# FelipeMartins96/rsoccer-isaac-cleanrl

Measured on NVIDIA B200. Metric: vss_env_steps_per_s, higher is better.
Workload: dtype f32

## Files before the change

### rsoccer_isaac_cleanrl_b200/csrc/vss_lane.cuh

```cuda
#pragma once
#include <stdint.h>
#include <math.h>
#include <string.h>
#if defined(__CUDACC__)
#include <cuda_bf16.h>
#endif

#include "../../include/vss_b200.h"

#if defined(__CUDACC__)
#define VSS_HD __host__ __device__ __forceinline__
#define VSS_HD_COLD inline __host__ __device__ __noinline__
#else
#define VSS_HD inline
#define VSS_HD_COLD inline
#endif

#ifndef VSS_INTEG_UNROLL
#define VSS_INTEG_UNROLL 1
#endif

namespace vss {

constexpr int INTEG_UNROLL = VSS_INTEG_UNROLL;
// ... 590 lines not shown
      const float p_dist = S[(W_PREV + 1 + r) * LDS];
      const float dist = norm2(fsub(x, bx), fsub(y, by));
      rew[4 * r + 2] = fmul(fsub(p_dist, dist), P.w_move);
    }
  }
  if (P.w_energy > 0.0f) {
#pragma unroll
    for (int r = 0; r < 6; ++r) {
      const float al = S[(11 + 9 * r) * LDS], ar = S[(12 + 9 * r) * LDS];
      rew[4 * r + 3] = fmul(-fmul(fadd(fabsf(al), fabsf(ar)), 0.5f), P.w_energy);
    }
  }
}

VSS_HD_COLD void reset_lane(float* S, const DevParams& P, const RngKey& key) {
  const uint32_t ep = fbits(S[VSS_W_EPISODE * LDS]);
  float px[7], py[7];
#pragma unroll 1
  for (uint32_t attempt = 0; attempt < (uint32_t)RESET_MAX_ATTEMPTS; ++attempt) {
    uint32_t u[16];
#pragma unroll
    for (uint32_t b = 0; b < 4; ++b) {
      const U4 g = rng_block(key, ep, STREAM_RESET_POS, (attempt << 2) | b);
      u[4 * b] = g.x; u[4 * b + 1] = g.y; u[4 * b + 2] = g.z; u[4 * b + 3] = g.w;
    }
#pragma unroll
    for (int e = 0; e < 7; ++e) {
      px[e] = fmul(fsub(u01(u[2 * e]), 0.5f), P.reset_sx);
      py[e] = fmul(fsub(u01(u[2 * e + 1]), 0.5f), P.reset_sy);
    }
    bool too_close = false;
#pragma unroll
    for (int a = 0; a < 7; ++a)
#pragma unroll
      for (int b = a + 1; b < 7; ++b) {
        const float dx = fsub(px[a], px[b]), dy = fsub(py[a], py[b]);
        too_close |= ffma(dy, dy, fmul(dx, dx)) < P.min_d2;
      }
    if (!too_close) break;
  }
  const U4 m0 = rng_block(key, ep, STREAM_RESET_MISC, 0), m1 = rng_block(key, ep, STREAM_RESET_MISC, 1);
  const uint32_t m[8] = {m0.x, m0.y, m0.z, m0.w, m1.x, m1.y, m1.z, m1.w};
  S[0] = px[0]; S[LDS] = py[0];
  S[2 * LDS] = fmul(fsub(u01(m[6]), 0.5f), P.ball_speed);
  S[3 * LDS] = fmul(fsub(u01(m[7]), 0.5f), P.ball_speed);
#pragma unroll
  for (int r = 0; r < 6; ++r) {
    float* b = S + (4 + 9 * r) * LDS;
    const float yaw = fsub(fmul(u01(m[r]), 6.283185307179586f), 3.141592653589793f);
    b[0] = px[1 + r]; b[LDS] = py[1 + r];
    b[2 * LDS] = 0.0f; b[3 * LDS] = 0.0f;
    b[4 * LDS] = cosf(yaw); b[5 * LDS] = sinf(yaw);
    b[6 * LDS] = 0.0f; b[7 * LDS] = 0.0f; b[8 * LDS] = 0.0f;
  }
  S[VSS_W_EPISODE * LDS] = bitsf(ep + 1u);
}

VSS_HD void ou_block(float a4[4], const DevParams& P, const RngKey& key, uint32_t step, uint32_t b) {
  const U4 g = rng_block(key, step, STREAM_OU, b);
  const uint32_t u[4] = {g.x, g.y, g.z, g.w};
#pragma unroll
  for (int h = 0; h < 2; ++h) {
    const float rad = fsqrt(fmul(-2.0f, logf(u01_open(u[2 * h]))));
    const float ang = fmul(6.283185307179586f, u01(u[2 * h + 1]));
    const float z[2] = {fmul(rad, cosf(ang)), fmul(rad, sinf(ang))};
#pragma unroll
    for (int c = 0; c < 2; ++c) {
      float& v = a4[2 * h + c];
      v = clampf(fadd(fsub(v, fmul(P.ou_theta, v)), fmul(P.ou_sigma, z[c])), -1.0f, 1.0f);
    }
  }
}
VSS_HD void ou_lane(float a[VSS_ACT_PER_FIELD], const DevParams& P, const RngKey& key, uint32_t step) {
#pragma unroll
  for (uint32_t b = 0; b < 3; ++b) ou_block(a + 4 * b, P, key, step, b);
}


#if defined(__CUDA_ARCH__)
VSS_HD F4 ld4(const float* p) { const float4 v = *reinterpret_cast<const float4*>(p); return F4{v.x, v.y, v.z, v.w}; }
VSS_HD void st4(float* p, const F4& v) { *reinterpret_cast<float4*>(p) = make_float4(v.x, v.y, v.z, v.w); }
VSS_HD void st4_stream(float* p, const F4& v) { __stcs(reinterpret_cast<float4*>(p), make_float4(v.x, v.y, v.z, v.w)); }
VSS_HD float ldg(const float* p) { return __ldg(p); }
VSS_HD void st_bf16x4(void* base, long long off, const F4& v) {
  const uint32_t lo = (uint32_t)__bfloat16_as_ushort(__float2bfloat16_rn(v.x)) |
                      ((uint32_t)__bfloat16_as_ushort(__float2bfloat16_rn(v.y)) << 16);
  const uint32_t hi = (uint32_t)__bfloat16_as_ushort(__float2bfloat16_rn(v.z)) |
                      ((uint32_t)__bfloat16_as_ushort(__float2bfloat16_rn(v.w)) << 16);
  *reinterpret_cast<uint2*>(reinterpret_cast<unsigned short*>(base) + off) = make_uint2(lo, hi);
}
#else
VSS_HD F4 ld4(const float* p) { return F4{p[0], p[1], p[2], p[3]}; }
VSS_HD void st4(float* p, const F4& v) { p[0] = v.x; p[1] = v.y; p[2] = v.z; p[3] = v.w; }
VSS_HD void st4_stream(float* p, const F4& v) { st4(p, v); }
VSS_HD float ldg(const float* p) { return *p; }
VSS_HD uint32_t bf16_rne(float f) {
  const uint32_t u = fbits(f);
  if ((u & 0x7FFFFFFFu) > 0x7F800000u) return 0x7FFFu;
  return (u + 0x7FFFu + ((u >> 16) & 1u)) >> 16;
}
VSS_HD void st_bf16x4(void* base, long long off, const F4& v) {
  unsigned short* p = reinterpret_cast<unsigned short*>(base) + off;
  p[0] = (unsigned short)bf16_rne(v.x); p[1] = (unsigned short)bf16_rne(v.y);
  p[2] = (unsigned short)bf16_rne(v.z); p[3] = (unsigned short)bf16_rne(v.w);
}
#endif

constexpr int VIEW_FULL = -1;
constexpr int VIEW_MATCH = 3;

struct StepArgs {
  float* state; long long n, ld; unsigned long long goff;
  long long env_begin;
  uint32_t seed_lo, seed_hi;
  unsigned long long* step_ctr;
  uint32_t grid;
  const float* actions;
  const float* inject;
  long long* reset_buf;
  float* obs;
  float* term_obs;
  float* rew;
  uint8_t* timeout;
  float* progress_f;
  const float* policy_action; float* action_buf; float* reward_v; long long* done_v;
  float* ep_ret; int* ep_len; float* ret_ret; int* ret_len;
  void* obs_bf16; float* done_f; float* timeout_f;
  void* packed;
  int fpw;
  int stagger_ns;
  int team_mode[2];
  const float* team_action[2];
  void* team_rows[2];
  long long count_envs, n_matches;
  vss_match_board* board;
};

template <int VIEW>
struct ViewShape {
  static constexpr int F4_PER = (VIEW == VIEW_FULL || VIEW == VIEW_MATCH) ? F4_PER_FIELD
                                                                          : (VIEW == VSS_VIEW_DMA ? 3 * F4_PER_ROW : F4_PER_ROW);
  static constexpr int AGENTS = VIEW == VSS_VIEW_DMA ? 3 : 1;
};

VSS_HD uint32_t step_index(const StepArgs& a) {
#if defined(__CUDA_ARCH__)
  return (uint32_t)__ldcg(a.step_ctr);
#else
  return (uint32_t)*a.step_ctr;
#endif
}

VSS_HD RngKey make_key(const StepArgs& a, long long env) {
  const unsigned long long gid = a.goff + (unsigned long long)env;
  return RngKey{a.seed_lo, a.seed_hi, (uint32_t)gid, (uint32_t)(gid >> 32)};
}

VSS_HD void load_state(float* S, const float* state, long long ld, long long env) {
  const float* src = state + env;
#pragma unroll
  for (int w = 0; w < VSS_STATE_WORDS; ++w) S[w * LDS] = ldg(src + (long long)w * ld);
}
VSS_HD void store_state(const float* S, float* state, long long ld, long long env) {
  float* dst = state + env;
#pragma unroll
  for (int w = 0; w < VSS_STATE_WORDS; ++w) dst[(long long)w * ld] = S[w * LDS];
}

VSS_HD bool match_needs_ou(const StepArgs& a) {
  return a.team_mode[0] == VSS_TEAM_OU || a.team_mode[0] == VSS_TEAM_SA || a.team_mode[1] == VSS_TEAM_OU ||
         a.team_mode[1] == VSS_TEAM_SA;
}
VSS_HD float match_slot(const StepArgs& a, long long env, int s, float prev, float ou) {
  const int t = s >= 6 ? 1 : 0, k = s - 6 * t;
  switch (a.team_mode[t]) {
    case VSS_TEAM_ZERO: return fmul(prev, 0.0f);
    case VSS_TEAM_OU: return ou;
    case VSS_TEAM_SA: return k < 2 ? a.team_action[t][2 * env + k] : ou;
    case VSS_TEAM_CMA:
    case VSS_TEAM_DMA: return a.team_action[t][6 * env + k];
    default: return prev;
  }
}

template <int VIEW>
VSS_HD void lane_phase1a(float* S, long long env, const StepArgs& a, const DevParams& P, const RngKey& key) {
  load_state(S, a.state, a.ld, env);
  float act[VSS_ACT_PER_FIELD];
  {
    const float* ap = (VIEW == VIEW_FULL ? a.actions : a.action_buf) + env * VSS_ACT_PER_FIELD;
#pragma unroll
    for (int q = 0; q < 3; ++q) {
      const F4 v = ld4(ap + 4 * q);
      act[4 * q] = v.x; act[4 * q + 1] = v.y; act[4 * q + 2] = v.z; act[4 * q + 3] = v.w;
    }
  }
  if (VIEW == VIEW_MATCH) {
    float ou[VSS_ACT_PER_FIELD];
#pragma unroll
    for (int q = 0; q < VSS_ACT_PER_FIELD; ++q) ou[q] = act[q];
    if (match_needs_ou(a)) ou_lane(ou, P, key, step_index(a));
#pragma unroll
    for (int q = 0; q < VSS_ACT_PER_FIELD; ++q) act[q] = match_slot(a, env, q, act[q], ou[q]);
    float* ap = a.action_buf + env * VSS_ACT_PER_FIELD;
#pragma unroll
    for (int q = 0; q < 3; ++q) st4(ap + 4 * q, F4{act[4 * q], act[4 * q + 1], act[4 * q + 2], act[4 * q + 3]});
  } else if (VIEW != VIEW_FULL) {
    ou_lane(act, P, key, step_index(a));
    if (VIEW == VSS_VIEW_SA) {
      act[0] = a.policy_action[2 * env]; act[1] = a.policy_action[2 * env + 1];
    } else {
#pragma unroll
      for (int q = 0; q < 6; ++q) act[q] = a.policy_action[6 * env + q];
    }
    float* ap = a.action_buf + env * VSS_ACT_PER_FIELD;
#pragma unroll
    for (int q = 0; q < 3; ++q) st4(ap + 4 * q, F4{act[4 * q], act[4 * q + 1], act[4 * q + 2], act[4 * q + 3]});
  }
  if (a.reset_buf[env] != 0) S[VSS_W_PROGRESS * LDS] = bitsf(0u);
#pragma unroll
  for (int r = 0; r < 6; ++r) {
    S[(11 + 9 * r) * LDS] = clampf(act[2 * r], -1.0f, 1.0f);
    S[(12 + 9 * r) * LDS] = clampf(act[2 * r + 1], -1.0f, 1.0f);
  }
  {
    const float pbx = S[0], pby = S[LDS];
    S[W_PREV * LDS] = ball_potential(pbx, pby, P.HL);
#pragma unroll
    for (int r = 0; r < 6; ++r)
      S[(W_PREV + 1 + r) * LDS] = norm2(fsub(S[(4 + 9 * r) * LDS], pbx), fsub(S[(5 + 9 * r) * LDS], pby));
  }
}

VSS_HD void load_state_words(float* S, const float* state, long long ld, long long env, int w0, int wstep) {
  const float* src = state + env;
  for (int w = w0; w < VSS_STATE_WORDS; w += wstep) S[w * LDS] = ldg(src + (long long)w * ld);
}
VSS_HD void store_state_words(const float* S, float* state, long long ld, long long env, int w0, int wstep) {
  float* dst = state + env;
  for (int w = w0; w < VSS_STATE_WORDS; w += wstep) dst[(long long)w * ld] = S[w * LDS];
}
template <int VIEW>
VSS_HD void actions_block(float* S, long long env, const StepArgs& a, const DevParams& P, const RngKey& key, int b) {
  float* ab = const_cast<float*>(VIEW == VIEW_FULL ? a.actions : a.action_buf) + env * VSS_ACT_PER_FIELD + 4 * b;
  const F4 v = ld4(ab);
  float act[4] = {v.x, v.y, v.z, v.w};
  if (VIEW == VIEW_MATCH) {
    float ou[4] = {v.x, v.y, v.z, v.w};
    if (match_needs_ou(a)) ou_block(ou, P, key, step_index(a), (uint32_t)b);
#pragma unroll
    for (int q = 0; q < 4; ++q) act[q] = match_slot(a, env, 4 * b + q, act[q], ou[q]);
    st4(ab, F4{act[0], act[1], act[2], act[3]});
  } else if (VIEW != VIEW_FULL) {
    ou_block(act, P, key, step_index(a), (uint32_t)b);
    if (VIEW == VSS_VIEW_SA) {
      if (b == 0) { act[0] = a.policy_action[2 * env]; act[1] = a.policy_action[2 * env + 1]; }
    } else {
      for (int q = 4 * b; q < 6 && q < 4 * b + 4; ++q) act[q - 4 * b] = a.policy_action[6 * env + q];
    }
    st4(ab, F4{act[0], act[1], act[2], act[3]});
  }
#pragma unroll
  for (int k = 0; k < 2; ++k) {
    const int r = 2 * b + k;
    S[(11 + 9 * r) * LDS] = clampf(act[2 * k], -1.0f, 1.0f);
    S[(12 + 9 * r) * LDS] = clampf(act[2 * k + 1], -1.0f, 1.0f);
  }
}
VSS_HD void prev_term_body(float* S, int body, const DevParams& P) {
  const float pbx = S[0], pby = S[LDS];
// ... 281 lines not shown
```

### rsoccer_isaac_cleanrl_b200/csrc/vss_step.cu

```cuda
#include <cuda_runtime.h>

#include <cstdio>
#include <cstdlib>
#include <cstring>
#include <new>
#include <string>

#include "vss_lane.cuh"

namespace vss {

__constant__ ObsTable c_obs_table = make_obs_table();

constexpr int TAB_WORDS = 80;
constexpr int CTR_WORDS = 4;

__host__ __device__ constexpr size_t smem_words(int wpb) {
  return TAB_WORDS + (size_t)wpb * TILE_WORDS + CTR_WORDS;
}


template <bool SYNC>
__device__ __forceinline__ void physics_tile(float* T, uint8_t* queue, int lane, bool active, const DevParams& P) {
  float* S = T + lane;
#pragma unroll 1
  for (int it = 0; it < P.substeps; ++it) {
    if (SYNC) __syncthreads();
    uint32_t m = active ? substep_pre_lane(S, P) : 0u;
    const int cnt = __popc(m);
    int incl = cnt;
#pragma unroll
    for (int d = 1; d < 32; d <<= 1) {
      const int v = __shfl_up_sync(0xffffffffu, incl, d);
      if (lane >= d) incl += v;
    }
    const int total = __shfl_sync(0xffffffffu, incl, 31);
    int pos = incl - cnt;
    while (m) {
      const int r = __ffs((int)m) - 1;
      m &= m - 1;
      queue[pos++] = (uint8_t)((lane << 3) | r);
    }
    __syncwarp();
#pragma unroll 1
    for (int t0 = 0; t0 < total; t0 += 32) {
      if (t0 + lane < total) {
        const int q = queue[t0 + lane];
        robot_walls_task(T + (q >> 3), q & 7, P);
      }
    }
    __syncwarp();
    if (active) substep_ball_walls_lane(S, P);
  }
}

__device__ __forceinline__ unsigned long long globaltimer_ns() {
  unsigned long long t;
  asm volatile("mov.u64 %0, %globaltimer;" : "=l"(t));
  return t;
}

template <int VIEW>
__device__ __forceinline__ void step_done(const StepArgs& a, uint32_t* ctr) {
  if (VIEW == VIEW_MATCH) __threadfence();
  __syncwarp();
  if ((threadIdx.x & 31) == 0 && atomicAdd(&ctr[3], 1u) == (blockDim.x >> 5) - 1u) {
    if (VIEW == VIEW_MATCH) __threadfence();
    unsigned long long* done_ctas = a.step_ctr + 1;
    if (atomicAdd(done_ctas, 1ull) == (unsigned long long)a.grid - 1ull) {
      if (VIEW == VIEW_MATCH) {
        __threadfence();
        board_close_step(a.board, a.n_matches);
      }
      atomicExch(done_ctas, 0ull);
      atomicAdd(a.step_ctr, 1ull);
    }
  }
}

template <int VIEW, bool INJECT, bool SYNC>
__global__ void __launch_bounds__(384)
k_step(const __grid_constant__ StepArgs a, const __grid_constant__ DevParams P) {
  extern __shared__ __align__(16) float smem[];
  uint32_t* tab = reinterpret_cast<uint32_t*>(smem);
  for (int i = threadIdx.x; i < F4_PER_FIELD; i += blockDim.x) tab[i] = c_obs_table.v[i];
  float* tiles = smem + TAB_WORDS;
  uint32_t* queue = reinterpret_cast<uint32_t*>(tiles + (blockDim.x >> 5) * TILE_STATE_WORDS);
  uint32_t* ctr = queue + (blockDim.x >> 5) * QUEUE_WORDS;
  if (threadIdx.x == 0) ctr[3] = 0u;
  if (a.stagger_ns > 0 && blockIdx.x < 148u * 6u) {
    const unsigned wait_ns = ((blockIdx.x / 148u) % 6u) * (unsigned)a.stagger_ns;
    const unsigned long long t0 = globaltimer_ns();
    while (globaltimer_ns() - t0 < wait_ns) __nanosleep(1000);
  }
  __syncthreads();
  const int lane = threadIdx.x & 31, warp = threadIdx.x >> 5;
  const long long tile = (long long)blockIdx.x * (blockDim.x >> 5) + warp;
  const long long env0 = a.env_begin + tile * a.fpw;
  if (!SYNC && env0 >= a.n) { if (VIEW != VIEW_FULL) step_done<VIEW>(a, ctr); return; }
  float* T = tiles + warp * TILE_STATE_WORDS;
  float* S = T + lane;
  const long long env = env0 + lane;
  const bool active = lane < a.fpw && env < a.n;
  const int valid = (int)max(0LL, min((long long)a.fpw, a.n - env0));
  constexpr int PER_FIELD = ViewShape<VIEW>::F4_PER;
  const RngKey key = make_key(a, env);
  if (active) lane_phase1a<VIEW>(S, env, a, P, key);
  if (INJECT) { if (active) lane_inject(S, env, a); }
  else physics_tile<SYNC>(T, reinterpret_cast<uint8_t*>(queue + warp * QUEUE_WORDS), lane, active, P);
  if (SYNC) __syncthreads();
  int code = LANE_RUNNING;
  if (active) code = lane_phase1d<VIEW>(S, env, a, P, key);
  const bool done = code == LANE_DONE;
  __syncwarp();
  if (SYNC) __syncthreads();
  const uint32_t done_mask = __ballot_sync(0xffffffffu, done);
  float* ob = a.obs + env0 * (PER_FIELD * 4);
  float* tob = a.term_obs ? a.term_obs + env0 * (PER_FIELD * 4) : nullptr;
  void* obh = (VIEW != VIEW_FULL && a.obs_bf16)
                  ? static_cast<void*>(static_cast<unsigned short*>(a.obs_bf16) + env0 * (ViewShape<VIEW>::AGENTS * 64))
                  : nullptr;
  void* pk = (VIEW != VIEW_FULL && a.packed)
                 ? static_cast<void*>(static_cast<char*>(a.packed) + env0 * (ViewShape<VIEW>::AGENTS * VSS_PACKED_ROW_BYTES))
                 : nullptr;
  if (VIEW == VIEW_MATCH) {}
  else if (PER_FIELD >= 32) write_obs_tile_rows<PER_FIELD>(T, tab, lane, valid, tob, ob, done_mask, obh, pk);
  else write_obs_tile(T, tab, lane, valid, PER_FIELD, tob, ob, done_mask, obh, pk);
  __syncwarp();
  if (done) reset_lane(S, P, key);
  __syncwarp();
  if (VIEW == VIEW_MATCH) write_match_tile(T, tab, lane, valid, env0, a);
  else write_obs_fields(T, tab, lane, PER_FIELD, ob, done_mask, obh, pk);
  if (SYNC) __syncthreads();
  if (active) lane_phase5<VIEW>(S, env, a, code != LANE_RUNNING);
  if (VIEW != VIEW_FULL) step_done<VIEW>(a, ctr);
}

__device__ __forceinline__ void body_barrier(int W) {
  asm volatile("bar.sync 1, %0;" ::"r"(W * 32) : "memory");
}

#ifdef VSS_PHASE_PROFILE
__device__ unsigned long long g_phase_prof[65536 * 8];
__device__ unsigned long long g_integ_prof[4096 * 16];
#define PROF_DECL unsigned long long pf_t = clock64(), pf_acc[7] = {0, 0, 0, 0, 0, 0, 0}; const unsigned long long pf_t0 = pf_t;
#define PROF_MARK(i) do { const unsigned long long pf_n = clock64(); pf_acc[i] += pf_n - pf_t; pf_t = pf_n; } while (0)
#define PROF_STORE do { if (threadIdx.x == 0 && blockIdx.x < 65536) { pf_acc[6] = clock64() - pf_t0; \
    for (int i = 0; i < 7; ++i) g_phase_prof[blockIdx.x * 8 + i] = pf_acc[i]; } } while (0)
#else
#define PROF_DECL
#define PROF_MARK(i)
#define PROF_STORE
#endif

template <int VIEW, bool INJECT>
__global__ void __launch_bounds__(32 * MAX_WPT)
k_step_cta(const __grid_constant__ StepArgs a, const __grid_constant__ DevParams P) {
  extern __shared__ __align__(16) float smem[];
  uint32_t* tab = reinterpret_cast<uint32_t*>(smem);
  for (int i = threadIdx.x; i < F4_PER_FIELD; i += blockDim.x) tab[i] = c_obs_table.v[i];
  float* T = smem + TAB_WORDS;
  uint32_t* ctr = reinterpret_cast<uint32_t*>(T + TILE_CTA_WORDS);
  const int lane = threadIdx.x & 31, warp = threadIdx.x >> 5, NW = blockDim.x >> 5, W = NW - 1;
  const bool helper = warp == W;
  if (threadIdx.x == 0) ctr[3] = 0u;
  const long long env0 = a.env_begin + (long long)blockIdx.x * a.fpw;
  float* S = T + lane;
  float* Sh = S + W_SHADOW * LDS;
  const long long env = env0 + lane;
  const bool active = lane < a.fpw && env < a.n;
  const int valid = (int)max(0LL, min((long long)a.fpw, a.n - env0));
  constexpr int PER_FIELD = ViewShape<VIEW>::F4_PER;
  const RngKey key = make_key(a, env);
  PROF_DECL
  if (active) load_state_words(S, a.state, a.ld, env, warp, NW);
  __syncthreads();
  if (active && !helper) {
    for (int b = warp; b < 3; b += W) actions_block<VIEW>(S, env, a, P, key, b);
    if (warp == 3 % W && a.reset_buf[env] != 0) S[VSS_W_PROGRESS * LDS] = bitsf(0u);
    for (int b = warp; b < 7; b += W) prev_term_body(S, b, P);
  }
  __syncthreads();
  PROF_MARK(0);
  if (helper && active) {
    Sh[VSS_W_EPISODE * LDS] = S[VSS_W_EPISODE * LDS];
    reset_lane(Sh, P, key);
  }
  if (INJECT) {
    if (warp == 0 && active) lane_inject(S, env, a);
  } else {
    if (!helper) {
#pragma unroll 1
      for (int it = 0; it < P.substeps; ++it) {
#ifdef VSS_PHASE_PROFILE
        const unsigned long long ig0 = clock64();
#endif
        if (active)
          for (int b = warp; b < 7; b += W) { if (b < 6) integrate_robot(S, b, P); else integrate_ball(S, P); }
#ifdef VSS_PHASE_PROFILE
        const unsigned long long ig1 = clock64();
#endif
        body_barrier(W);
#ifdef VSS_PHASE_PROFILE
        if (lane == 0 && blockIdx.x < 4096) {
          const unsigned long long ig2 = clock64();
          if (it == 0) { g_integ_prof[blockIdx.x * 16 + warp] = 0; g_integ_prof[blockIdx.x * 16 + 8 + warp] = 0; }
          g_integ_prof[blockIdx.x * 16 + warp] += ig1 - ig0;
          g_integ_prof[blockIdx.x * 16 + 8 + warp] += ig2 - ig1;
        }
#endif
        PROF_MARK(1);
        {
          uint32_t m = 0u;
          if (active)
            for (int q = warp; q < 21; q += W) m |= broadphase_pair(S, q, P);
          S[(W_SCR + warp) * LDS] = bitsf(m);
        }
        body_barrier(W);
// ... 80 lines not shown
  if (active) {
    load_state(S, state, ld, env);
    flagged = reset_buf[env] != 0;
    if (flagged) {
      const unsigned long long gid = goff + (unsigned long long)env;
      reset_lane(S, P, RngKey{seed_lo, seed_hi, (uint32_t)gid, (uint32_t)(gid >> 32)});
      store_state(S, state, ld, env);
    }
  }
  __syncwarp();
  if (obs) write_obs_tile(T, tab, lane, valid, F4_PER_FIELD, nullptr, obs + env0 * VSS_OBS_PER_FIELD, 0u);
}

struct GaeRows { float r, v, nv, d, to; };

__device__ __forceinline__ GaeRows gae_load(const float* __restrict__ rewards, const float* __restrict__ values,
                                            const float* __restrict__ next_values, const float* __restrict__ next_dones,
                                            const float* __restrict__ next_timeouts, long long i) {
  return GaeRows{__ldg(rewards + i), __ldg(values + i), __ldg(next_values + i), __ldg(next_dones + i),
                 __ldg(next_timeouts + i)};
}

__device__ __forceinline__ float gae_step(const GaeRows& x, float last, float gamma, float gamma_lambda,
                                          float* __restrict__ advantages, float* __restrict__ returns, long long i) {
  const float nnt = (x.d != 0.0f && !(x.to != 0.0f)) ? 0.0f : 1.0f;
  const float delta = fsub(fadd(x.r, fmul(fmul(gamma, x.nv), nnt)), x.v);
  last = fadd(delta, fmul(fmul(gamma_lambda, fsub(1.0f, x.d)), last));
  advantages[i] = last;
  returns[i] = fadd(last, x.v);
  return last;
}

template <bool PREFETCH>
__global__ void __launch_bounds__(128)
k_gae(const float* __restrict__ rewards, const float* __restrict__ values, const float* __restrict__ next_values,
      const float* __restrict__ next_dones, const float* __restrict__ next_timeouts,
      float* __restrict__ advantages, float* __restrict__ returns, int T, long long N, float gamma,
      float gamma_lambda) {
  const long long n = (long long)blockIdx.x * blockDim.x + threadIdx.x;
  if (n >= N) return;
  float last = 0.0f;
  constexpr int U = 8;
  int t = T - 1;
  if (t >= U - 1) {
    GaeRows cur[U], nxt[U];
#pragma unroll
    for (int k = 0; k < U; ++k)
      cur[k] = gae_load(rewards, values, next_values, next_dones, next_timeouts, (long long)(t - k) * N + n);
    for (; t >= U - 1; t -= U) {
      const bool more = t - U >= U - 1;
      if (PREFETCH && more) {
#pragma unroll
        for (int k = 0; k < U; ++k)
          nxt[k] = gae_load(rewards, values, next_values, next_dones, next_timeouts, (long long)(t - U - k) * N + n);
      }
#pragma unroll
      for (int k = 0; k < U; ++k)
        last = gae_step(cur[k], last, gamma, gamma_lambda, advantages, returns, (long long)(t - k) * N + n);
      if (more) {
#pragma unroll
        for (int k = 0; k < U; ++k)
          cur[k] = PREFETCH ? nxt[k]
                            : gae_load(rewards, values, next_values, next_dones, next_timeouts,
                                       (long long)(t - U - k) * N + n);
      }
    }
  }
  for (; t >= 0; --t) {
    const long long i = (long long)t * N + n;
    last = gae_step(gae_load(rewards, values, next_values, next_dones, next_timeouts, i), last, gamma, gamma_lambda,
                    advantages, returns, i);
  }
}

}

using namespace vss;

struct vss_engine {
  int device;
  int64_t n, ld, goff;
  uint64_t seed;
  unsigned long long* d_step;
  vss_params params;
  DevParams dp;
  float* state;
  void* aux_obs_bf16; float* aux_done_f; float* aux_timeout_f;
  void* packed_rows;
  int wpt_override;
  int fpt_override;
  int64_t range_first, range_count;
  cudaStream_t host_stream[2];
  cudaEvent_t host_start, host_done[2];
  bool host_ready;
};

static thread_local std::string g_last_error;

static int fail(int code, const char* what, cudaError_t e = cudaSuccess) {
  g_last_error = what;
  if (e != cudaSuccess) { g_last_error += ": "; g_last_error += cudaGetErrorString(e); }
  return code;
}
#define VSS_CUDA(call)                                        \
  do {                                                        \
    cudaError_t e_ = (call);                                  \
    if (e_ != cudaSuccess) return fail(VSS_E_CUDA, #call, e_); \
  } while (0)

struct LaunchShape {
  int wpb, fpw, stagger_ns, wpt;
  bool sync;
  unsigned grid;
  size_t smem;
};

static int auto_wpt(int64_t n) {
  const int64_t tiles = (n + 31) / 32;
  return tiles <= 256 ? 8 : 1;
}

static int auto_cta_fields(int64_t n) { return n <= 148 * 8 ? 8 : (n <= 148 * 16 ? 16 : 32); }

static LaunchShape launch_shape(int64_t n, bool step_kernel = true, int wpt_override = 0, int fpt_override = 0) {
  LaunchShape s;
  s.wpt = !step_kernel ? 1 : (wpt_override > 0 ? wpt_override : auto_wpt(n));
  if (s.wpt > 1) {
    s.wpb = s.wpt; s.sync = true; s.stagger_ns = 0;
    s.fpw = fpt_override > 0 ? fpt_override : auto_cta_fields(n);
    s.grid = (unsigned)((n + s.fpw - 1) / s.fpw);
    s.smem = sizeof(float) * (TAB_WORDS + TILE_CTA_WORDS + CTR_WORDS);
    return s;
  }
  s.fpw = !step_kernel ? 32 : (fpt_override > 0 ? fpt_override : (n < 148 * 40 ? 8 : (n < 148 * 192 ? 16 : 32)));
  const int64_t tiles = (n + s.fpw - 1) / s.fpw;
  s.wpb = tiles < 148 * 2 ? 1 : (tiles < 148 * 20 ? 2 : 4);
  s.sync = s.wpb == 4;
  s.grid = (unsigned)((tiles + s.wpb - 1) / s.wpb);
  s.smem = sizeof(float) * smem_words(s.wpb);
  s.stagger_ns = (s.sync && s.grid > 148u * 6u) ? 5000 : 0;
  return s;
}

static int use_device(vss_handle h) {
  int cur = -1;
  VSS_CUDA(cudaGetDevice(&cur));
  if (cur != h->device) VSS_CUDA(cudaSetDevice(h->device));
  return VSS_OK;
}

static StepArgs base_args(vss_handle h) {
  StepArgs a;
  memset(&a, 0, sizeof(a));
  a.state = h->state; a.n = h->n; a.ld = h->ld; a.goff = (unsigned long long)h->goff;
  a.seed_lo = (uint32_t)h->seed; a.seed_hi = (uint32_t)(h->seed >> 32); a.step_ctr = h->d_step;
  return a;
}

template <int VIEW, bool INJECT>
static int launch_step(vss_handle h, StepArgs a, void* stream) {
  const LaunchShape ls = launch_shape(h->n, true, h->wpt_override, h->fpt_override);
  a.fpw = ls.fpw; a.stagger_ns = ls.stagger_ns;
  a.grid = ls.grid;
  unsigned grid = ls.grid;
  if (h->range_count > 0) {
    const int64_t per_cta = ls.wpt > 1 ? ls.fpw : (int64_t)ls.wpb * ls.fpw;
    if (h->range_first % per_cta != 0 || (h->range_count % per_cta != 0 && h->range_first + h->range_count != h->n))
      return fail(VSS_E_INVALID, "step range: first / count must be multiples of vss_step_granularity()");
    a.env_begin = h->range_first;
    a.n = h->range_first + h->range_count;
    grid = (unsigned)((h->range_count + per_cta - 1) / per_cta);
  }
  if (ls.wpt > 1) k_step_cta<VIEW, INJECT><<<grid, ls.wpt * 32, ls.smem, (cudaStream_t)stream>>>(a, h->dp);
  else if (ls.sync) k_step<VIEW, INJECT, true><<<grid, ls.wpb * 32, ls.smem, (cudaStream_t)stream>>>(a, h->dp);
  else k_step<VIEW, INJECT, false><<<grid, ls.wpb * 32, ls.smem, (cudaStream_t)stream>>>(a, h->dp);
  VSS_CUDA(cudaGetLastError());
  return VSS_OK;
}

extern "C" {

VSS_API const char* vss_last_error(void) { return g_last_error.c_str(); }
VSS_API const char* vss_version(void) { return "vss_b200 0.1 (sm_100a)"; }

VSS_API int vss_default_params(vss_params* p) {
  if (!p) return fail(VSS_E_INVALID, "vss_default_params: null");
  const double PI = 3.14159265358979323846;
  p->dt = 0.05f; p->substeps = 4; p->max_episode_length = 400;
  p->field_half_length = 0.75f; p->field_half_width = 0.65f; p->goal_half_width = 0.2f; p->goal_depth = 0.1f;
  p->ball_radius = 0.02134f;
  p->ball_mass = (float)(1130.0 * 4.0 / 3.0 * PI * 0.02134 * 0.02134 * 0.02134);
  p->ball_drag = (float)(0.5 * 2.0 / 7.0);
  p->robot_half_size = 0.035f; p->robot_mass = 0.44f;
  p->robot_inertia = (float)(0.4 * (0.07 * 0.07 + 0.07 * 0.07) / 12.0 + 2.0 * 0.02 * 0.03375 * 0.03375);
  p->wheel_radius = 0.024f; p->wheel_half_track = 0.03375f; p->wheel_coll_radius = 0.024f;
  p->max_wheel_rad_s = 42.0f; p->drive_damping = 0.01f; p->drive_max_torque = 0.1f;
  p->wheel_inertia = (float)(0.0002 + 0.4 * 0.02 * 0.024 * 0.024);
  p->mu_traction = 0.7f; p->mu_lateral = 0.55f; p->gravity = 9.81f;
  p->restitution = 0.0f; p->mu_ball_robot = 0.5f; p->mu_ball_wall = 1.0f; p->mu_robot_wall = 0.5f;
  p->reset_scale_x = (float)(1.5 - 0.14); p->reset_scale_y = (float)(1.3 - 0.14);
  p->min_placement_dist = 0.07f; p->ball_reset_speed = 1.0f;
  p->w_goal = 10.0f; p->w_grad = 2.0f; p->w_move = 3.0f; p->w_energy = 0.0f;
  p->ou_theta = 0.1f; p->ou_sigma = 0.15f;
  return VSS_OK;
}

VSS_API int vss_create(vss_handle* out, const vss_params* p, int64_t num_envs, int64_t global_env_offset,
                       int device, uint64_t seed) {
  if (!out || !p) return fail(VSS_E_INVALID, "vss_create: null argument");
  if (num_envs <= 0) return fail(VSS_E_INVALID, "vss_create: num_envs must be > 0");
  if (p->substeps < 0 || p->substeps > 64) return fail(VSS_E_INVALID, "vss_create: substeps out of range");
  int count = 0;
  cudaError_t e = cudaGetDeviceCount(&count);
  if (e != cudaSuccess || count == 0)
    return fail(VSS_E_NODEVICE, "vss_create: no CUDA device (this library has no CPU fallback)", e);
  if (device < 0 || device >= count) return fail(VSS_E_INVALID, "vss_create: bad device index");
  cudaDeviceProp prop;
  VSS_CUDA(cudaGetDeviceProperties(&prop, device));
  if (prop.major != 10)
    return fail(VSS_E_NODEVICE, "vss_create: kernels are built for sm_100a only (Blackwell B200)");
  VSS_CUDA(cudaSetDevice(device));
  vss_engine* h = new (std::nothrow) vss_engine();
  if (!h) return fail(VSS_E_NOMEM, "vss_create: host allocation failed");
  h->device = device; h->n = num_envs; h->ld = (num_envs + 31) / 32 * 32; h->goff = global_env_offset;
  h->aux_obs_bf16 = nullptr; h->aux_done_f = nullptr; h->aux_timeout_f = nullptr; h->packed_rows = nullptr;
  h->range_first = 0; h->range_count = 0; h->wpt_override = 0; h->fpt_override = 0; h->host_ready = false;
  h->seed = seed; h->d_step = nullptr; h->params = *p; h->dp = derive_params(*p); h->state = nullptr;
  const size_t bytes = sizeof(float) * VSS_STATE_WORDS * (size_t)h->ld;
  e = cudaMalloc(&h->state, bytes);
  if (e != cudaSuccess) { delete h; return fail(VSS_E_NOMEM, "vss_create: cudaMalloc(state)", e); }
  e = cudaMemset(h->state, 0, bytes);
  if (e == cudaSuccess) e = cudaMalloc(&h->d_step, 3 * sizeof(unsigned long long));
  if (e == cudaSuccess) e = cudaMemset(h->d_step, 0, 3 * sizeof(unsigned long long));
  if (e != cudaSuccess) { cudaFree(h->state); cudaFree(h->d_step); delete h; return fail(VSS_E_CUDA, "vss_create: cudaMemset", e); }
  *out = h;
  return VSS_OK;
}

VSS_API int vss_destroy(vss_handle h) {
  if (!h) return VSS_OK;
  if (h->host_ready) {
    for (int i = 0; i < 2; ++i) { cudaStreamDestroy(h->host_stream[i]); cudaEventDestroy(h->host_done[i]); }
    cudaEventDestroy(h->host_start);
  }
  cudaFree(h->state);
  cudaFree(h->d_step);
  delete h;
  return VSS_OK;
}

VSS_API int64_t vss_num_envs(vss_handle h) { return h ? h->n : 0; }
VSS_API int64_t vss_state_ld(vss_handle h) { return h ? h->ld : 0; }
VSS_API uint64_t vss_step_count(vss_handle h) {
  if (!h) return 0;
  unsigned long long v = 0;
  if (use_device(h) != VSS_OK) return 0;
  if (cudaMemcpy(&v, h->d_step, sizeof(v), cudaMemcpyDeviceToHost) != cudaSuccess) return 0;
  return v;
}
VSS_API uint64_t vss_sanitised_count(vss_handle h) {
  if (!h) return 0;
  unsigned long long v = 0;
  if (use_device(h) != VSS_OK) return 0;
  if (cudaMemcpy(&v, h->d_step + 2, sizeof(v), cudaMemcpyDeviceToHost) != cudaSuccess) return 0;
  return v;
}
VSS_API int vss_set_step_count(vss_handle h, uint64_t n) {
  if (!h) return fail(VSS_E_INVALID, "null handle");
  if (int rc = use_device(h)) return rc;
  if (n > 0xFFFFFFFFull) return fail(VSS_E_INVALID, "vss_set_step_count: the step index is a 32-bit counter");
  const unsigned long long v[2] = {(unsigned long long)n, 0ull};
  VSS_CUDA(cudaMemcpy(h->d_step, v, sizeof(v), cudaMemcpyHostToDevice));
  return VSS_OK;
}

VSS_API int vss_set_reward_weights(vss_handle h, const float w[4]) {
  if (!h || !w) return fail(VSS_E_INVALID, "vss_set_reward_weights: null");
  h->params.w_goal = w[0]; h->params.w_grad = w[1]; h->params.w_move = w[2]; h->params.w_energy = w[3];
  h->dp.w_goal = w[0]; h->dp.w_grad = w[1]; h->dp.w_move = w[2]; h->dp.w_energy = w[3];
  return VSS_OK;
}

VSS_API int vss_reset_dones(vss_handle h, const int64_t* reset_buf, float* obs, void* stream) {
  if (!h || !reset_buf) return fail(VSS_E_INVALID, "vss_reset_dones: null argument");
  if (int rc = use_device(h)) return rc;
  const LaunchShape ls = launch_shape(h->n, false);
  k_reset_dones<<<ls.grid, ls.wpb * 32, ls.smem, (cudaStream_t)stream>>>(
      h->state, h->n, h->ld, (unsigned long long)h->goff, (uint32_t)h->seed, (uint32_t)(h->seed >> 32),
      reinterpret_cast<const long long*>(reset_buf), obs, h->dp);
  VSS_CUDA(cudaGetLastError());
  return VSS_OK;
}

VSS_API int vss_step(vss_handle h, const float* actions, int64_t* reset_buf, float* obs, float* term_obs,
                     float* rew, uint8_t* timeout, float* progress_f, void* stream) {
  if (!h || !actions || !reset_buf || !obs || !rew || !timeout)
    return fail(VSS_E_INVALID, "vss_step: null argument");
  if (int rc = use_device(h)) return rc;
  StepArgs a = base_args(h);
  a.actions = actions; a.reset_buf = reinterpret_cast<long long*>(reset_buf); a.obs = obs; a.term_obs = term_obs;
  a.rew = rew; a.timeout = timeout; a.progress_f = progress_f;
  return launch_step<VIEW_FULL, false>(h, a, stream);
}

VSS_API int vss_step_injected(vss_handle h, const float* actions, const float* post_state, int64_t* reset_buf,
                              float* obs, float* term_obs, float* rew, uint8_t* timeout, float* progress_f,
                              void* stream) {
  if (!h || !actions || !post_state || !reset_buf || !obs || !rew || !timeout)
    return fail(VSS_E_INVALID, "vss_step_injected: null argument");
  if (int rc = use_device(h)) return rc;
  StepArgs a = base_args(h);
  a.actions = actions; a.inject = post_state; a.reset_buf = reinterpret_cast<long long*>(reset_buf); a.obs = obs;
  a.term_obs = term_obs; a.rew = rew; a.timeout = timeout; a.progress_f = progress_f;
  return launch_step<VIEW_FULL, true>(h, a, stream);
}

VSS_API int vss_step_view(vss_handle h, int view, const float* policy_action, float* action_buf,
                          int64_t* reset_buf, float* obs_v, float* term_obs_v, float* rews_v, float* reward_v,
                          int64_t* done_v, uint8_t* timeout_v, float* progress_v, float* ep_ret, int32_t* ep_len,
                          float* ret_ret, int32_t* ret_len, void* stream) {
  if (!h || !policy_action || !action_buf || !reset_buf || !obs_v || !rews_v || !reward_v || !done_v || !timeout_v)
    return fail(VSS_E_INVALID, "vss_step_view: null argument");
  if (ep_ret && (!ep_len || !ret_ret || !ret_len))
    return fail(VSS_E_INVALID, "vss_step_view: episode statistics need all four buffers");
  if (int rc = use_device(h)) return rc;
  StepArgs a = base_args(h);
  a.policy_action = policy_action; a.action_buf = action_buf; a.reset_buf = reinterpret_cast<long long*>(reset_buf);
  a.obs = obs_v; a.term_obs = term_obs_v; a.rew = rews_v; a.reward_v = reward_v;
  a.done_v = reinterpret_cast<long long*>(done_v); a.timeout = timeout_v; a.progress_f = progress_v;
// ... 194 lines not shown
```

Measured before the change: 1.768 billion.

## Overlap consecutive step launches via programmatic dependent launch and per-CTA tickets

Launches the synchronous full-view step kernel with programmatic stream serialization so the next step's grid can start before the previous one finishes. Each CTA takes a ticket and spins on a per-CTA finished counter with acquire/release, so it only reads state after the same CTA of the prior launch has released it. State loads switch to L2-coherent loads, since the non-coherent path could return stale values. This targets the launch gap and tail between back-to-back steps, at the cost of spin-waiting, extra ticket memory, a host mutex, and a risk of deadlock if CTA scheduling order is unfavorable.

```diff
diff --git a/profiles/step_overlap_bench.py b/profiles/step_overlap_bench.py
--- /dev/null
+++ b/profiles/step_overlap_bench.py
@@ -0,0 +1,115 @@
+import argparse
+import ctypes as C
+import json
+import os
+import subprocess
+import sys
+
+import torch
+
+ROOT = os.path.dirname(os.path.dirname(os.path.abspath(__file__)))
+sys.path.insert(0, ROOT)
+from rsoccer_isaac_cleanrl_b200 import _lib
+from rsoccer_isaac_cleanrl_b200.envs import VSS, load_cfg
+
+SIZES = (262144, 1048576)
+STEPS = (20, 400)
+
+
+def load(path):
+    lib = C.CDLL(os.path.abspath(path))
+    for name, (res, args) in _lib._SYMBOLS.items():
+        fn = getattr(lib, name)
+        fn.restype, fn.argtypes = res, args
+    return lib
+
+
+def make_task(lib, n):
+    saved = _lib._lib
+    _lib._lib = lib
+    try:
+        cfg = load_cfg()
+        cfg["env"]["numEnvs"] = n
+        task = VSS(cfg, "cuda:0", "cuda:0", 0, True, seed=0)
+    finally:
+        _lib._lib = saved
+    task.reset_buf.zero_()
+    st = task.engine.get_state()
+    g = torch.Generator(device="cuda"); g.manual_seed(1234)
+    st[58, :n] = torch.randint(0, 400, (n,), device="cuda", generator=g, dtype=torch.int32).view(torch.float32)
+    task.engine.set_state(st)
+    acts = [torch.rand((n, 2, 3, 2), device="cuda", generator=g) * 2 - 1 for _ in range(4)]
+    return task, acts
+
+
+def time_us(task, acts, steps, warm=20):
+    for i in range(warm):
+        task.step(acts[i & 3])
+    torch.cuda.synchronize()
+    e0, e1 = torch.cuda.Event(enable_timing=True), torch.cuda.Event(enable_timing=True)
+    e0.record()
+    for i in range(steps):
+        task.step(acts[i & 3])
+    e1.record()
+    torch.cuda.synchronize()
+    return e0.elapsed_time(e1) * 1e3 / steps
+
+
+def card():
+    q = subprocess.run(["nvidia-smi", "--query-gpu=name,power.limit,clocks.max.sm", "--format=csv,noheader"],
+                       capture_output=True, text=True)
+    return q.stdout.strip() or torch.cuda.get_device_name(0)
+
+
+def main():
+    ap = argparse.ArgumentParser()
+    ap.add_argument("--lib", action="append", default=[], metavar="LABEL=PATH")
+    ap.add_argument("--reps", type=int, default=5)
+    args = ap.parse_args()
+    libs = {}
+    if os.environ.get("VSS_AB_LIB"):
+        libs["parent"] = os.environ["VSS_AB_LIB"]
+    libs["new"] = _lib.LIB_PATH
+    libs.update(x.split("=", 1) for x in args.lib)
+    libs = {k: os.path.relpath(p, ROOT) for k, p in libs.items()}
+    bound = {k: load(os.path.join(ROOT, p)) for k, p in libs.items()}
+    print(f"card: {card()}")
+    print("libs: " + ", ".join(f"{k} = {p}" for k, p in libs.items()))
+    res = {k: {f"{n}x{s}": [] for n in SIZES for s in STEPS} for k in libs}
+    for n in SIZES:
+        tasks = {k: make_task(lib, n) for k, lib in bound.items()}
+        for rep in range(args.reps):
+            for s in STEPS:
+                for k, (task, acts) in tasks.items():
+                    res[k][f"{n}x{s}"].append(time_us(task, acts, s))
+        del tasks
+        torch.cuda.empty_cache()
+    print("us per step: median [min, max] over repetitions")
+    print(f"{'build':8s} " + " ".join(f"{f'{n} x {s}':>26s}" for n in SIZES for s in STEPS)
+          + "   fixed us/launch (20, 400 steps)")
+    summary = {}
+    for k in libs:
+        cells, med = [], {}
+        for n in SIZES:
+            for s in STEPS:
+                v = sorted(res[k][f"{n}x{s}"])
+                med[(n, s)] = v[len(v) // 2]
+                cells.append(f"{med[(n, s)]:8.1f} [{v[0]:7.1f}, {v[-1]:7.1f}]")
+        fixed = []
+        for s in STEPS:
+            b = (med[(SIZES[1], s)] - med[(SIZES[0], s)]) / (SIZES[1] - SIZES[0])
+            fixed.append(med[(SIZES[0], s)] - b * SIZES[0])
+        summary[k] = {"median_us": {f"{n}x{s}": med[(n, s)] for n in SIZES for s in STEPS},
+                      "fixed_us_per_launch": dict(zip(map(str, STEPS), fixed))}
+        print(f"{k:8s} " + " ".join(cells) + f"   {fixed[0]:6.1f} {fixed[1]:6.1f}")
+    if "parent" in libs:
+        for k in libs:
+            if k != "parent":
+                print(f"{k} vs parent, speed-up of the median: " + " ".join(
+                    f"{n}x{s}: {summary['parent']['median_us'][f'{n}x{s}'] / summary[k]['median_us'][f'{n}x{s}']:.3f}"
+                    for n in SIZES for s in STEPS))
+    print(json.dumps({"card": card(), "libs": libs, "reps": args.reps, "raw_us": res, "summary": summary}))
+
+
+if __name__ == "__main__":
+    main()
diff --git a/rsoccer_isaac_cleanrl_b200/csrc/vss_lane.cuh b/rsoccer_isaac_cleanrl_b200/csrc/vss_lane.cuh
--- a/rsoccer_isaac_cleanrl_b200/csrc/vss_lane.cuh
+++ b/rsoccer_isaac_cleanrl_b200/csrc/vss_lane.cuh
@@ -696,6 +696,7 @@
 VSS_HD void st4(float* p, const F4& v) { *reinterpret_cast<float4*>(p) = make_float4(v.x, v.y, v.z, v.w); }
 VSS_HD void st4_stream(float* p, const F4& v) { __stcs(reinterpret_cast<float4*>(p), make_float4(v.x, v.y, v.z, v.w)); }
 VSS_HD float ldg(const float* p) { return __ldg(p); }
+VSS_HD float ldcg(const float* p) { return __ldcg(p); }
 VSS_HD void st_bf16x4(void* base, long long off, const F4& v) {
   const uint32_t lo = (uint32_t)__bfloat16_as_ushort(__float2bfloat16_rn(v.x)) |
                       ((uint32_t)__bfloat16_as_ushort(__float2bfloat16_rn(v.y)) << 16);
@@ -708,6 +709,7 @@
 VSS_HD void st4(float* p, const F4& v) { p[0] = v.x; p[1] = v.y; p[2] = v.z; p[3] = v.w; }
 VSS_HD void st4_stream(float* p, const F4& v) { st4(p, v); }
 VSS_HD float ldg(const float* p) { return *p; }
+VSS_HD float ldcg(const float* p) { return *p; }
 VSS_HD uint32_t bf16_rne(float f) {
   const uint32_t u = fbits(f);
   if ((u & 0x7FFFFFFFu) > 0x7F800000u) return 0x7FFFu;
@@ -748,6 +750,8 @@
   void* team_rows[2];
   long long count_envs, n_matches;
   vss_match_board* board;
+  uint32_t* started;
+  uint32_t* finished;
 };
 
 template <int VIEW>
@@ -770,10 +774,11 @@
   return RngKey{a.seed_lo, a.seed_hi, (uint32_t)gid, (uint32_t)(gid >> 32)};
 }
 
+template <bool COHERENT = false>
 VSS_HD void load_state(float* S, const float* state, long long ld, long long env) {
   const float* src = state + env;
 #pragma unroll
-  for (int w = 0; w < VSS_STATE_WORDS; ++w) S[w * LDS] = ldg(src + (long long)w * ld);
+  for (int w = 0; w < VSS_STATE_WORDS; ++w) S[w * LDS] = COHERENT ? ldcg(src + (long long)w * ld) : ldg(src + (long long)w * ld);
 }
 VSS_HD void store_state(const float* S, float* state, long long ld, long long env) {
   float* dst = state + env;
@@ -797,9 +802,9 @@
   }
 }
 
-template <int VIEW>
+template <int VIEW, bool COHERENT = false>
 VSS_HD void lane_phase1a(float* S, long long env, const StepArgs& a, const DevParams& P, const RngKey& key) {
-  load_state(S, a.state, a.ld, env);
+  load_state<COHERENT>(S, a.state, a.ld, env);
   float act[VSS_ACT_PER_FIELD];
   {
     const float* ap = (VIEW == VIEW_FULL ? a.actions : a.action_buf) + env * VSS_ACT_PER_FIELD;
diff --git a/rsoccer_isaac_cleanrl_b200/csrc/vss_step.cu b/rsoccer_isaac_cleanrl_b200/csrc/vss_step.cu
--- a/rsoccer_isaac_cleanrl_b200/csrc/vss_step.cu
+++ b/rsoccer_isaac_cleanrl_b200/csrc/vss_step.cu
@@ -3,6 +3,7 @@
 #include <cstdio>
 #include <cstdlib>
 #include <cstring>
+#include <mutex>
 #include <new>
 #include <string>
 
@@ -78,9 +79,19 @@
   }
 }
 
+__device__ __forceinline__ uint32_t ld_acquire_gpu(const uint32_t* p) {
+  uint32_t v;
+  asm volatile("ld.acquire.gpu.global.u32 %0, [%1];" : "=r"(v) : "l"(p) : "memory");
+  return v;
+}
+__device__ __forceinline__ void st_release_gpu(uint32_t* p, uint32_t v) {
+  asm volatile("st.release.gpu.global.u32 [%0], %1;" ::"l"(p), "r"(v) : "memory");
+}
+
 template <int VIEW, bool INJECT, bool SYNC>
 __global__ void __launch_bounds__(384)
 k_step(const __grid_constant__ StepArgs a, const __grid_constant__ DevParams P) {
+  constexpr bool OVERLAP = VIEW == VIEW_FULL && !INJECT && SYNC;
   extern __shared__ __align__(16) float smem[];
   uint32_t* tab = reinterpret_cast<uint32_t*>(smem);
   for (int i = threadIdx.x; i < F4_PER_FIELD; i += blockDim.x) tab[i] = c_obs_table.v[i];
@@ -88,12 +99,19 @@
   uint32_t* queue = reinterpret_cast<uint32_t*>(tiles + (blockDim.x >> 5) * TILE_STATE_WORDS);
   uint32_t* ctr = queue + (blockDim.x >> 5) * QUEUE_WORDS;
   if (threadIdx.x == 0) ctr[3] = 0u;
-  if (a.stagger_ns > 0 && blockIdx.x < 148u * 6u) {
+  if (OVERLAP) {
+    if (threadIdx.x == 0) {
+      const uint32_t g = atomicAdd(a.started + blockIdx.x, 1u);
+      while (ld_acquire_gpu(a.finished + blockIdx.x) != g) __nanosleep(256);
+      ctr[0] = g;
+    }
+  } else if (a.stagger_ns > 0 && blockIdx.x < 148u * 6u) {
     const unsigned wait_ns = ((blockIdx.x / 148u) % 6u) * (unsigned)a.stagger_ns;
     const unsigned long long t0 = globaltimer_ns();
     while (globaltimer_ns() - t0 < wait_ns) __nanosleep(1000);
   }
   __syncthreads();
+  if (OVERLAP) asm volatile("griddepcontrol.launch_dependents;" ::: "memory");
   const int lane = threadIdx.x & 31, warp = threadIdx.x >> 5;
   const long long tile = (long long)blockIdx.x * (blockDim.x >> 5) + warp;
   const long long env0 = a.env_begin + tile * a.fpw;
@@ -105,7 +123,7 @@
   const int valid = (int)max(0LL, min((long long)a.fpw, a.n - env0));
   constexpr int PER_FIELD = ViewShape<VIEW>::F4_PER;
   const RngKey key = make_key(a, env);
-  if (active) lane_phase1a<VIEW>(S, env, a, P, key);
+  if (active) lane_phase1a<VIEW, OVERLAP>(S, env, a, P, key);
   if (INJECT) { if (active) lane_inject(S, env, a); }
   else physics_tile<SYNC>(T, reinterpret_cast<uint8_t*>(queue + warp * QUEUE_WORDS), lane, active, P);
   if (SYNC) __syncthreads();
@@ -134,6 +152,13 @@
   if (SYNC) __syncthreads();
   if (active) lane_phase5<VIEW>(S, env, a, code != LANE_RUNNING);
   if (VIEW != VIEW_FULL) step_done<VIEW>(a, ctr);
+  if (OVERLAP) {
+    __syncthreads();
+    if (threadIdx.x == 0) {
+      __threadfence();
+      st_release_gpu(a.finished + blockIdx.x, ctr[0] + 1u);
+    }
+  }
 }
 
 __device__ __forceinline__ void body_barrier(int W) {
@@ -380,6 +405,7 @@
   int64_t n, ld, goff;
   uint64_t seed;
   unsigned long long* d_step;
+  uint32_t* tickets;
   vss_params params;
   DevParams dp;
   float* state;
@@ -452,7 +478,41 @@
   memset(&a, 0, sizeof(a));
   a.state = h->state; a.n = h->n; a.ld = h->ld; a.goff = (unsigned long long)h->goff;
   a.seed_lo = (uint32_t)h->seed; a.seed_hi = (uint32_t)(h->seed >> 32); a.step_ctr = h->d_step;
+  a.started = h->tickets; a.finished = h->tickets + h->ld / 32;
   return a;
+}
+
+struct OverlapKey {
+  vss_handle h;
+  cudaStream_t stream;
+  int64_t per_cta;
+  unsigned long long capture;
+  bool operator==(const OverlapKey& o) const {
+    return h == o.h && stream == o.stream && per_cta == o.per_cta && capture == o.capture;
+  }
+};
+static std::mutex g_overlap_mu;
+static OverlapKey g_last_overlap{};
+
+static int launch_step_overlapped(vss_handle h, const StepArgs& a, unsigned grid, const LaunchShape& ls, cudaStream_t st) {
+  cudaStreamCaptureStatus cs = cudaStreamCaptureStatusNone;
+  unsigned long long cid = 0;
+  VSS_CUDA(cudaStreamGetCaptureInfo(st, &cs, &cid));
+  const int64_t per_cta = (int64_t)ls.wpb * ls.fpw;
+  const OverlapKey key{h, st, per_cta, cs == cudaStreamCaptureStatusActive ? cid : 0ull};
+  StepArgs b = a;
+  b.started += a.env_begin / per_cta; b.finished += a.env_begin / per_cta;
+  std::lock_guard<std::mutex> lock(g_overlap_mu);
+  cudaLaunchAttribute attr;
+  attr.id = cudaLaunchAttributeProgrammaticStreamSerialization;
+  attr.val.programmaticStreamSerializationAllowed = g_last_overlap == key ? 1 : 0;
+  cudaLaunchConfig_t cfg = {};
+  cfg.gridDim = dim3(grid); cfg.blockDim = dim3(ls.wpb * 32); cfg.dynamicSmemBytes = ls.smem; cfg.stream = st;
+  cfg.attrs = &attr; cfg.numAttrs = 1;
+  g_last_overlap = OverlapKey{};
+  VSS_CUDA(cudaLaunchKernelEx(&cfg, k_step<VIEW_FULL, false, true>, b, h->dp));
+  g_last_overlap = key;
+  return VSS_OK;
 }
 
 template <int VIEW, bool INJECT>
@@ -470,6 +530,7 @@
     grid = (unsigned)((h->range_count + per_cta - 1) / per_cta);
   }
   if (ls.wpt > 1) k_step_cta<VIEW, INJECT><<<grid, ls.wpt * 32, ls.smem, (cudaStream_t)stream>>>(a, h->dp);
+  else if (VIEW == VIEW_FULL && !INJECT && ls.sync) return launch_step_overlapped(h, a, grid, ls, (cudaStream_t)stream);
   else if (ls.sync) k_step<VIEW, INJECT, true><<<grid, ls.wpb * 32, ls.smem, (cudaStream_t)stream>>>(a, h->dp);
   else k_step<VIEW, INJECT, false><<<grid, ls.wpb * 32, ls.smem, (cudaStream_t)stream>>>(a, h->dp);
   VSS_CUDA(cudaGetLastError());
@@ -523,14 +584,19 @@
   h->device = device; h->n = num_envs; h->ld = (num_envs + 31) / 32 * 32; h->goff = global_env_offset;
   h->aux_obs_bf16 = nullptr; h->aux_done_f = nullptr; h->aux_timeout_f = nullptr; h->packed_rows = nullptr;
   h->range_first = 0; h->range_count = 0; h->wpt_override = 0; h->fpt_override = 0; h->host_ready = false;
-  h->seed = seed; h->d_step = nullptr; h->params = *p; h->dp = derive_params(*p); h->state = nullptr;
+  h->seed = seed; h->d_step = nullptr; h->tickets = nullptr; h->params = *p; h->dp = derive_params(*p); h->state = nullptr;
   const size_t bytes = sizeof(float) * VSS_STATE_WORDS * (size_t)h->ld;
   e = cudaMalloc(&h->state, bytes);
   if (e != cudaSuccess) { delete h; return fail(VSS_E_NOMEM, "vss_create: cudaMalloc(state)", e); }
   e = cudaMemset(h->state, 0, bytes);
   if (e == cudaSuccess) e = cudaMalloc(&h->d_step, 3 * sizeof(unsigned long long));
   if (e == cudaSuccess) e = cudaMemset(h->d_step, 0, 3 * sizeof(unsigned long long));
-  if (e != cudaSuccess) { cudaFree(h->state); cudaFree(h->d_step); delete h; return fail(VSS_E_CUDA, "vss_create: cudaMemset", e); }
+  if (e == cudaSuccess) e = cudaMalloc(&h->tickets, 2 * sizeof(uint32_t) * (size_t)(h->ld / 32));
+  if (e == cudaSuccess) e = cudaMemset(h->tickets, 0, 2 * sizeof(uint32_t) * (size_t)(h->ld / 32));
+  if (e != cudaSuccess) {
+    cudaFree(h->state); cudaFree(h->d_step); cudaFree(h->tickets); delete h;
+    return fail(VSS_E_CUDA, "vss_create: cudaMemset", e);
+  }
   *out = h;
   return VSS_OK;
 }
@@ -543,6 +609,11 @@
   }
   cudaFree(h->state);
   cudaFree(h->d_step);
+  cudaFree(h->tickets);
+  {
+    std::lock_guard<std::mutex> lock(g_overlap_mu);
+    if (g_last_overlap.h == h) g_last_overlap = OverlapKey{};
+  }
   delete h;
   return VSS_OK;
 }
```

Result: faster. 1.803 billion (median of 6 runs) (+2.0%).
